# HKUST-Aerial-Robotics/MIND

Hardware: AMD Instinct MI355X
Metric: sim steps/sec (whole node) + scenario-tree nodes expanded/sec, AV2 demo scenes (higher is better)
Workload: dtype f32-class (bf16 hi+mid+lo split operands = 24 significand bits, six products, fp32 accumulate) pair kernel + ActorNet, f32 elsewhere in the predictor, f64 iLQR

## Files before the change

### mind_amd/csrc/actor_mfma_kernels.hip

```cpp
#include <hip/hip_runtime.h>
#include <stdint.h>

#define AM_T 1024
#ifdef MIND_ACTOR_TRACE
__device__ long long am_tr_[64];
__device__ int am_trn_;
#define AM_MARK() do { if (blockIdx.x == 0 && threadIdx.x == 0) { const long long n_ = clock64(); am_tr_[am_trn_ & 63] = n_; ++am_trn_; } } while (0)
#else
#define AM_MARK() do {} while (0)
#endif
#define AM_WAVES 16
#define AM_MAXT 2
#define AM_RSD(C) (3 * (C) / 2 + 4)
#define AM_BUF 2496
#define AM_XIN 0
#define AM_O0 1344
#define AM_FA (AM_O0 + 7 * AM_BUF)
#define AM_RED (AM_FA + 48 * AM_RSD(128))
#define AM_LDS_DWORDS (AM_RED + 64)

struct AmRes { const u32 *c1, *c2, *ds; const float *g1, *b1, *g2, *b2, *gd, *bd; };
struct AmLat { const u32 *w; const float *g, *b; };
struct AmW {
  AmRes res[9];
  AmLat lat[4];
};
typedef u32 u32x2 __attribute__((ext_vector_type(2)));

__device__ __forceinline__ float am_block_sum(float v, float *red, int flip) {
  v = wave_sum(v);
  float *r = red + (flip & 1) * 32;
  if ((threadIdx.x & 63) == 0) r[threadIdx.x >> 6] = v;
  __syncthreads();
  float s = 0.f;
#pragma unroll
  for (int w = 0; w < AM_WAVES; ++w) s += r[w];
  return s;
}

template <int NP>
__device__ __forceinline__ void am_store_split(u32 *rowp, int plane, const f32x4 &y) {
  u32x2 h, m, l;
  h[0] = pk_bf16(y[0], y[1]); h[1] = pk_bf16(y[2], y[3]);
  *(u32x2 *)rowp = h;
  if (NP == 1) return;
  const float r0 = y[0] - bf_lo_f32(h[0]), r1 = y[1] - bf_hi_f32(h[0]), r2 = y[2] - bf_lo_f32(h[1]), r3 = y[3] - bf_hi_f32(h[1]);
  m[0] = pk_bf16(r0, r1); m[1] = pk_bf16(r2, r3);
  *(u32x2 *)(rowp + plane) = m;
  l[0] = pk_bf16(r0 - bf_lo_f32(m[0]), r1 - bf_hi_f32(m[0])); l[1] = pk_bf16(r2 - bf_lo_f32(m[1]), r3 - bf_hi_f32(m[1]));
// ... 39 lines not shown
      const int row = t * STRIDE + dk - PAD;
      u32x4 bh = {0u, 0u, 0u, 0u}, bm = {0u, 0u, 0u, 0u}, bl = {0u, 0u, 0u, 0u};
      if (dk < KSZ && t < Tout && row >= 0 && row < Tin) {
        const u32 *bp = in + row * RSD + (ci >> 1);
        bh = *(const u32x4 *)bp;
        if (NP >= 3) bm = *(const u32x4 *)(bp + PLANE);
        if (NP == 6) bl = *(const u32x4 *)(bp + 2 * PLANE);
      }
      acc[i] = MFMA_BF(ah, bh, acc[i]);
      if (NP >= 3) {
        if (NP == 6) {
          corr = MFMA_BF(al, bh, corr);
          corr = MFMA_BF(ah, bl, corr);
          corr = MFMA_BF(am, bm, corr);
        }
        corr = MFMA_BF(am, bh, corr);
        corr = MFMA_BF(ah, bm, corr);
      }
    }
    if (NP >= 3) acc[i] += corr;
  }
}

template <int NP>
__device__ __forceinline__ void am_gn(f32x4 (&acc)[AM_MAXT], int Cout, int Tout, const float *__restrict__ g,
                                      const float *__restrict__ b, const u32 *resid, const float *up, bool relu, u32 *outs,
                                      float *outf, float *__restrict__ gout, float *red) {
  const int lane = threadIdx.x & 63, wave = threadIdx.x >> 6;
  const int r = lane & 15, q = lane >> 4;
  const int ntt = (Tout + 15) >> 4;
  const int tiles = (Cout >> 4) * ntt;
  const int RSD = AM_RSD(Cout), PLANE = Cout >> 1;
  f32x4 gg[AM_MAXT], bb[AM_MAXT];
  float s = 0.f;
#pragma unroll
  for (int i = 0; i < AM_MAXT; ++i) {
    const int ti = wave + AM_WAVES * i;
    if (ti >= tiles) continue;
    const int mt = ti / ntt, nt = ti - mt * ntt;
    gg[i] = *(const f32x4 *)(g + mt * 16 + q * 4);
    bb[i] = *(const f32x4 *)(b + mt * 16 + q * 4);
    if (nt * 16 + r < Tout) s += (acc[i][0] + acc[i][1]) + (acc[i][2] + acc[i][3]);
  }
  const float n = (float)(Cout * Tout);
  const float mean = am_block_sum(s, red, 0) / n;
  float v = 0.f;
// ... 56 lines not shown
  AM_MARK();
  const u32 *resid = in;
  if (DS) {
    am_conv<NP, LGCI, 1, STRIDE>(in, Tin, W.ds, Cout, Tout, acc);
    AM_MARK();
    am_gn<NP>(acc, Cout, Tout, W.gd, W.bd, nullptr, nullptr, false, t2, nullptr, nullptr, red);
    AM_MARK();
    resid = t2;
  }
  am_conv<NP, LGCO, 3, 1>(t1, Tout, W.c2, Cout, Tout, acc);
  AM_MARK();
  am_gn<NP>(acc, Cout, Tout, W.g2, W.b2, resid, nullptr, true, out, nullptr, nullptr, red);
  AM_MARK();
}

template <int NP, int LGC>
__device__ __forceinline__ void am_lateral(const u32 *src, int T, const AmLat &W, const float *up, float *dstf, u32 *dsts,
                                           float *red) {
  f32x4 acc[AM_MAXT];
  am_conv<NP, LGC, 3, 1>(src, T, W.w, 128, T, acc);
  AM_MARK();
  am_gn<NP>(acc, 128, T, W.g, W.b, nullptr, up, false, dsts, dstf, nullptr, red);
  AM_MARK();
}

template <int NP>
__global__ __launch_bounds__(AM_T) void k_actor_mfma(const float *__restrict__ actors , int n_actors,
                                                     float *__restrict__ out , AmW W) {
  extern __shared__ __attribute__((aligned(16))) u32 smu[];
  u32 *xin = smu + AM_XIN;
  u32 *o0 = smu + AM_O0, *o1 = o0 + AM_BUF, *o2 = o1 + AM_BUF, *o3 = o2 + AM_BUF;
  u32 *ta = o3 + AM_BUF, *tb = ta + AM_BUF, *tc = tb + AM_BUF;
  u32 *fa = smu + AM_FA;
  float *red = (float *)(smu + AM_RED);
  const int tid = threadIdx.x;
  const int a = blockIdx.x;
  if (a >= n_actors) return;
  if (tid < 48 * 8) {
    const int t = tid >> 3, c = (tid & 7) * 2;
    const float v0 = c < 14 ? actors[((size_t)a * 14 + c) * 48 + t] : 0.f;
    const float v1 = c + 1 < 14 ? actors[((size_t)a * 14 + c + 1) * 48 + t] : 0.f;
    u32 *p = xin + t * AM_RSD(16) + (c >> 1);
    const u32 h = pk_bf16(v0, v1);
    const float r0 = v0 - bf_lo_f32(h), r1 = v1 - bf_hi_f32(h);
    const u32 m = pk_bf16(r0, r1);
    p[0] = h; p[8] = m; p[16] = pk_bf16(r0 - bf_lo_f32(m), r1 - bf_hi_f32(m));
  }
  __syncthreads();
#ifdef MIND_ACTOR_TRACE
  if (blockIdx.x == 0 && tid == 0) am_trn_ = 0;
#endif
  AM_MARK();
  am_res<NP, 4, 5, 1, true>(xin, 48, W.res[0], ta, tb, tc, red);
  am_res<NP, 5, 5, 1, false>(ta, 48, W.res[1], o0, tb, tc, red);
  am_res<NP, 5, 6, 2, true>(o0, 48, W.res[2], ta, tb, tc, red);
  am_res<NP, 6, 6, 1, false>(ta, 24, W.res[3], o1, tb, tc, red);
  am_res<NP, 6, 7, 2, true>(o1, 24, W.res[4], ta, tb, tc, red);
  am_res<NP, 7, 7, 1, false>(ta, 12, W.res[5], o2, tb, tc, red);
  am_res<NP, 7, 8, 2, true>(o2, 12, W.res[6], ta, tb, tc, red);
  am_res<NP, 8, 8, 1, false>(ta, 6, W.res[7], o3, tb, tc, red);
  am_lateral<NP, 8>(o3, 6, W.lat[3], nullptr, (float *)ta, nullptr, red);
  am_lateral<NP, 7>(o2, 12, W.lat[2], (const float *)ta, (float *)tb, nullptr, red);
  am_lateral<NP, 6>(o1, 24, W.lat[1], (const float *)tb, (float *)o2, nullptr, red);
  am_lateral<NP, 5>(o0, 48, W.lat[0], (const float *)o2, nullptr, fa, red);
  {
    const AmRes &R = W.res[8];
    f32x4 acc[AM_MAXT];
    am_conv<NP, 7, 3, 1>(fa, 48, R.c1, 128, 48, acc);
    AM_MARK();
    am_gn<NP>(acc, 128, 48, R.g1, R.b1, nullptr, nullptr, true, o0, nullptr, nullptr, red);
    AM_MARK();
    am_conv<NP, 7, 3, 1>(o0, 48, R.c2, 128, 48, acc);
    AM_MARK();
    am_gn<NP>(acc, 128, 48, R.g2, R.b2, fa, nullptr, true, nullptr, nullptr, out + (size_t)a * 128, red);
    AM_MARK();
  }
#ifdef MIND_ACTOR_TRACE
  if (blockIdx.x == 0 && tid == 0) {
    printf("[k_actor_mfma<%d>] cycles conv/gn per stage:", NP);
    for (int q = 1; q < am_trn_ && q < 64; ++q) printf(" %lld", am_tr_[q] - am_tr_[q - 1]);
    printf("\n");
  }
#endif
}
extern "C" size_t mind_actor_mfma_lds_bytes() { return (size_t)AM_LDS_DWORDS * sizeof(u32); }
```

### mind_amd/csrc/mind_hip.hip

```cpp
#include <hip/hip_runtime.h>

#include <cmath>
#include <cstdarg>
#include <cstdio>
#include <cstdlib>
#include <algorithm>
#include <cstring>
#include <map>
#include <string>
#include <thread>
#include <atomic>
#include <functional>
#include <vector>

#include "../../include/mind_hip.h"
#include "encdec_kernels.hip"
#include "fusion_kernels.hip"
#include "pair_bf16_kernels.hip"
#include "pair_tile_kernels.hip"
#include "pair_tile6_kernels.hip"
#include "token_mfma_kernels.hip"
#include "actor_mfma_kernels.hip"
#include "actor_lw_kernels.hip"
#include "token_lw_kernels.hip"
// ... 239 lines not shown
  (void)hipFuncSetAttribute((const void *)k_pair_t6<1>, hipFuncAttributeMaxDynamicSharedMemorySize, (int)mind_pair_bf_lds_bytes());
  if (const char *te = getenv("MIND_PAIR_TILE")) c->pt.pair_tile = !(te[0] == '0');
  if (const char *xe = getenv("MIND_XCD_ORDER")) c->pt.xcd_order = !(xe[0] == '0');

  if (const char *pe = getenv("MIND_PAIR_PREC")) {
    const std::string v = pe;
    if (v == "f32" || v == "0") c->pair_prec = 0;
    else if (v == "bf16x3" || v == "1") c->pair_prec = 1;
    else if (v == "bf16" || v == "2") c->pair_prec = 2;
    else if (v == "bf16x6" || v == "3") c->pair_prec = 3;
  }
  (void)hipFuncSetAttribute((const void *)k_actor_net, hipFuncAttributeMaxDynamicSharedMemorySize, (int)mind_actor_lds_bytes());
  (void)hipFuncSetAttribute((const void *)k_actor_mfma<3>, hipFuncAttributeMaxDynamicSharedMemorySize, (int)mind_actor_mfma_lds_bytes());
  (void)hipFuncSetAttribute((const void *)k_actor_mfma<6>, hipFuncAttributeMaxDynamicSharedMemorySize, (int)mind_actor_mfma_lds_bytes());
  (void)hipFuncSetAttribute((const void *)k_dec_actor_mfma<1>, hipFuncAttributeMaxDynamicSharedMemorySize, (int)mind_dec_actor_mfma_lds_bytes());
  (void)hipFuncSetAttribute((const void *)k_dec_actor_mfma<3>, hipFuncAttributeMaxDynamicSharedMemorySize, (int)mind_dec_actor_mfma_lds_bytes());
  (void)hipFuncSetAttribute((const void *)k_dec_actor_mfma<6>, hipFuncAttributeMaxDynamicSharedMemorySize, (int)mind_dec_actor_mfma_lds_bytes());
  if (const char *se = getenv("MIND_ACTOR_SPLIT")) c->pt.actor_np = atoi(se) == 3 ? 3 : 6;
  (void)hipFuncSetAttribute((const void *)k_actor_mfma<1>, hipFuncAttributeMaxDynamicSharedMemorySize, (int)mind_actor_mfma_lds_bytes());
  if (const char *me = getenv("MIND_ENC_MFMA")) c->pt.enc_mfma = !(me[0] == '0');
  if (const char *me = getenv("MIND_ACTOR_F32")) c->pt.actor_f32 = !(me[0] == '0');
  if (const char *me = getenv("MIND_ACTOR_F32_MIN")) c->pt.actor_f32_min = atoi(me);
  if (const char *me = getenv("MIND_ACTOR_LW_MIN")) c->pt.actor_lw_min = atoi(me);
  lw_set_attributes();
  (void)hipFuncSetAttribute((const void *)k_actor_f32<1>, hipFuncAttributeMaxDynamicSharedMemorySize, (int)mind_actor_f32_lds_bytes(1));
  (void)hipFuncSetAttribute((const void *)k_actor_f32<2>, hipFuncAttributeMaxDynamicSharedMemorySize, (int)mind_actor_f32_lds_bytes(2));
  if (const char *de = getenv("MIND_DEC_MFMA_MIN")) c->pt.dec_mfma_min = atoi(de);
  if (const char *oe = getenv("MIND_DEC_OVERLAP")) c->pt.dec_overlap = !(oe[0] == '0');
  (void)hipFuncSetAttribute((const void *)k_ilqr<true, 0>, hipFuncAttributeMaxDynamicSharedMemorySize, (int)il_lds_bytes(0));
  (void)hipFuncSetAttribute((const void *)k_ilqr<false, 1>, hipFuncAttributeMaxDynamicSharedMemorySize, (int)il_lds_bytes(0));
  (void)hipFuncSetAttribute((const void *)k_ilqr<false, 0>, hipFuncAttributeMaxDynamicSharedMemorySize, (int)il_lds_bytes(0));
  (void)hipFuncSetAttribute((const void *)k_ilqr<false, 2>, hipFuncAttributeMaxDynamicSharedMemorySize, (int)il_lds_bytes(0));
  if (const char *te = getenv("MIND_TOK_MFMA")) c->pt.tok_mfma = !(te[0] == '0');
  if (const char *te = getenv("MIND_TOK_SMALL_MAX")) c->pt.tok_small_max = atoi(te);
  if (const char *te = getenv("MIND_TOK_MERGE")) c->pt.tok_merge = !(te[0] == '0');
  if (const char *te = getenv("MIND_DEC_MW")) c->pt.dec_mw = !(te[0] == '0');
  if (const char *te = getenv("MIND_DEC_CLS_SIDE")) c->pt.dec_cls_side = !(te[0] == '0');
  if (const char *te = getenv("MIND_TOK_BF_MIN_N")) c->pt.tok_bf_min_n = atoi(te);
  if (const char *te = getenv("MIND_TOK_LW_MIN_N")) c->pt.tok_lw_min_n = atoi(te);
  if (const char *te = getenv("MIND_TOK_LW_MIN")) c->pt.tok_lw_min = atoi(te);
  if (const char *te = getenv("MIND_TGT_SIDE")) c->pt.tgt_side = !(te[0] == '0');
  if (const char *te = getenv("MIND_PL_TAB_SIDE")) c->pl_tab_side = !(te[0] == '0');
  (void)hipFuncSetAttribute((const void *)k_token_mfma<0>, hipFuncAttributeMaxDynamicSharedMemorySize, (int)mind_token_mfma_lds_bytes());
  (void)hipFuncSetAttribute((const void *)k_token_mfma<1>, hipFuncAttributeMaxDynamicSharedMemorySize, (int)mind_token_mfma_lds_bytes());
  if (const char *ce = getenv("MIND_PLAN_CHUNK_MB")) { const long v = atol(ce); if (v > 0) c->plan_chunk_mb = v; }
  if (const char *we = getenv("MIND_TAB_SMALL")) c->tab_small = atoi(we) != 0;
// ... 470 lines not shown
  WeightBlob &B = c->blob;
  B.host.clear();
  B.off.clear();
  auto lin_ln = [&](const std::string &key, const std::string &p, int idx, int n_out, int n_in) {
    B.add(key + ".W", transpose(sd.get(p + "." + std::to_string(idx) + ".weight", (int64_t)n_out * n_in), n_out, n_in));
    B.add(key + ".b", vec(sd.get(p + "." + std::to_string(idx) + ".bias", n_out), n_out));
    B.add(key + ".g", vec(sd.get(p + "." + std::to_string(idx + 1) + ".weight", n_out), n_out));
    B.add(key + ".be", vec(sd.get(p + "." + std::to_string(idx + 1) + ".bias", n_out), n_out));
  };
  lin_ln("lane.proj", "lane_net.proj", 0, 128, 16);
  for (int b = 0; b < 2; ++b) {
    std::string p = "lane_net.aggre" + std::to_string(b + 1), k = "lane.a" + std::to_string(b);
    lin_ln(k + ".f10", p + ".fc1", 0, 128, 128);
    lin_ln(k + ".f13", p + ".fc1", 3, 128, 128);
    lin_ln(k + ".f20", p + ".fc2", 0, 128, 256);
    lin_ln(k + ".f23", p + ".fc2", 3, 128, 128);
    B.add(k + ".ng", vec(sd.get(p + ".norm.weight", 128), 128));
    B.add(k + ".nb", vec(sd.get(p + ".norm.bias", 128), 128));
  }
  {
    const int chans[4] = {32, 64, 128, 256};
    int n_in = 14;
    int ri = 0;
    auto res = [&](const std::string &p, int ci, int co, bool ds) {
      std::string k = "act.r" + std::to_string(ri++);
      B.add(k + ".c1", conv_t(sd.get(p + ".conv1.weight", (int64_t)co * ci * 3), co, ci, 3));
      B.add(k + ".c2", conv_t(sd.get(p + ".conv2.weight", (int64_t)co * co * 3), co, co, 3));
      B.add(k + ".c1B", pack_conv_frag(sd.get(p + ".conv1.weight", (int64_t)co * ci * 3), co, ci, 3));
      B.add(k + ".c2B", pack_conv_frag(sd.get(p + ".conv2.weight", (int64_t)co * co * 3), co, co, 3));
      B.add(k + ".c1F", pack_conv_f32(sd.get(p + ".conv1.weight", (int64_t)co * ci * 3), co, ci, 3));
      B.add(k + ".c2F", pack_conv_f32(sd.get(p + ".conv2.weight", (int64_t)co * co * 3), co, co, 3));
      B.add(k + ".g1", vec(sd.get(p + ".bn1.weight", co), co));
      B.add(k + ".b1", vec(sd.get(p + ".bn1.bias", co), co));
      B.add(k + ".g2", vec(sd.get(p + ".bn2.weight", co), co));
      B.add(k + ".b2", vec(sd.get(p + ".bn2.bias", co), co));
      if (ds) {
        B.add(k + ".ds", conv_t(sd.get(p + ".downsample.0.weight", (int64_t)co * ci), co, ci, 1));
        B.add(k + ".dsB", pack_conv_frag(sd.get(p + ".downsample.0.weight", (int64_t)co * ci), co, ci, 1));
        B.add(k + ".dsF", pack_conv_f32(sd.get(p + ".downsample.0.weight", (int64_t)co * ci), co, ci, 1));
        B.add(k + ".gd", vec(sd.get(p + ".downsample.1.weight", co), co));
        B.add(k + ".bd", vec(sd.get(p + ".downsample.1.bias", co), co));
      }
    };
    for (int g = 0; g < 4; ++g) {
      res("actor_net.groups." + std::to_string(g) + ".0", n_in, chans[g], true);
      res("actor_net.groups." + std::to_string(g) + ".1", chans[g], chans[g], false);
      n_in = chans[g];
    }
    res("actor_net.output", 128, 128, false);
    for (int g = 0; g < 4; ++g) {
      std::string p = "actor_net.lateral." + std::to_string(g), k = "act.lat" + std::to_string(g);
      B.add(k + ".W", conv_t(sd.get(p + ".conv.weight", (int64_t)128 * chans[g] * 3), 128, chans[g], 3));
      B.add(k + ".WB", pack_conv_frag(sd.get(p + ".conv.weight", (int64_t)128 * chans[g] * 3), 128, chans[g], 3));
      B.add(k + ".WF", pack_conv_f32(sd.get(p + ".conv.weight", (int64_t)128 * chans[g] * 3), 128, chans[g], 3));
      B.add(k + ".g", vec(sd.get(p + ".norm.weight", 128), 128));
      B.add(k + ".b", vec(sd.get(p + ".norm.bias", 128), 128));
    }
  }
  lin_ln("fus.pa", "fusion_net.proj_actor", 0, 128, 128);
  lin_ln("fus.pl", "fusion_net.proj_lane", 0, 128, 128);
  B.add("fus.pa.WM", pack_afrag(sd.get("fusion_net.proj_actor.0.weight", 128 * 128), 128));
  B.add("fus.pl.WM", pack_afrag(sd.get("fusion_net.proj_lane.0.weight", 128 * 128), 128));
  B.add("fus.pa.WB", pack_tok_bfrag(sd.get("fusion_net.proj_actor.0.weight", 128 * 128), 128));
  B.add("fus.pl.WB", pack_tok_bfrag(sd.get("fusion_net.proj_lane.0.weight", 128 * 128), 128));
  {
    const float *W = sd.get("fusion_net.proj_rpe_scene.0.weight", 128 * 5);
    const float *b = sd.get("fusion_net.proj_rpe_scene.0.bias", 128);
    const float *g = sd.get("fusion_net.proj_rpe_scene.1.weight", 128);
    const float *be = sd.get("fusion_net.proj_rpe_scene.1.bias", 128);
    std::vector<float> t(1024, 0.f);
    if (W && b && g && be)
      for (int ch = 0; ch < 32; ++ch)
        for (int w = 0; w < 4; ++w) {
          const int f = 4 * ch + w;
          for (int k = 0; k < 5; ++k) t[ch * 32 + k * 4 + w] = W[f * 5 + k];
          t[ch * 32 + 20 + w] = b[f];
          t[ch * 32 + 24 + w] = g[f];
          t[ch * 32 + 28 + w] = be[f];
        }
    B.add("fus.rtab", t);
// ... 146 lines not shown
  ActorW &aw = c->actorW;
  for (int r = 0; r < 9; ++r) {
    std::string k = "act.r" + std::to_string(r);
    aw.res[r].c1 = P(k + ".c1"); aw.res[r].g1 = P(k + ".g1"); aw.res[r].b1 = P(k + ".b1");
    aw.res[r].c2 = P(k + ".c2"); aw.res[r].g2 = P(k + ".g2"); aw.res[r].b2 = P(k + ".b2");
    aw.res[r].ds = P(k + ".ds"); aw.res[r].gd = P(k + ".gd"); aw.res[r].bd = P(k + ".bd");
  }
  for (int g = 0; g < 4; ++g) {
    std::string k = "act.lat" + std::to_string(g);
    aw.latW[g] = P(k + ".W"); aw.latG[g] = P(k + ".g"); aw.latB[g] = P(k + ".b");
  }
  AmW &bw = c->actorBW;
  for (int r = 0; r < 9; ++r) {
    std::string k = "act.r" + std::to_string(r);
    AmRes &R = bw.res[r];
    R.c1 = (const u32 *)P(k + ".c1B"); R.c2 = (const u32 *)P(k + ".c2B"); R.ds = (const u32 *)P(k + ".dsB");
    R.g1 = aw.res[r].g1; R.b1 = aw.res[r].b1; R.g2 = aw.res[r].g2; R.b2 = aw.res[r].b2;
    R.gd = aw.res[r].gd; R.bd = aw.res[r].bd;
  }
  for (int g = 0; g < 4; ++g) {
    bw.lat[g].w = (const u32 *)P("act.lat" + std::to_string(g) + ".WB");
    bw.lat[g].g = aw.latG[g]; bw.lat[g].b = aw.latB[g];
  }
  AfW &fw = c->actorFW;
  for (int r = 0; r < 9; ++r) {
    std::string k = "act.r" + std::to_string(r);
    AfRes &R = fw.res[r];
    R.c1 = P(k + ".c1F"); R.c2 = P(k + ".c2F"); R.ds = P(k + ".dsF");
    R.g1 = aw.res[r].g1; R.b1 = aw.res[r].b1; R.g2 = aw.res[r].g2; R.b2 = aw.res[r].b2;
    R.gd = aw.res[r].gd; R.bd = aw.res[r].bd;
  }
  for (int g = 0; g < 4; ++g) {
    fw.lat[g].w = P("act.lat" + std::to_string(g) + ".WF");
    fw.lat[g].g = aw.latG[g]; fw.lat[g].b = aw.latB[g];
  }
  c->rtab = P("fus.rtab");
  for (int L = 0; L < 6; ++L) {
    std::string k = "fus.L" + std::to_string(L);
    c->WAe[L] = P(k + ".WAe");
    c->WAp[L] = P(k + ".WAp");
    c->WBe[L] = (const u32 *)P(k + ".WBe");
    c->WBp[L] = (const u32 *)P(k + ".WBp");
    c->WLe[L] = (const u32 *)P(k + ".WLe");
    c->WLp[L] = (const u32 *)P(k + ".WLp");
    c->vtab[L] = P(k + ".vtab");
  }
// ... 447 lines not shown
```

### mind_amd/csrc/pred_choice.h

```cpp
#pragma once
#include <cstring>
#include <vector>

struct PredTuning {
  bool pair_tile = true;
  bool xcd_order = true;
  bool enc_mfma = true;
  int actor_np = 6;
  bool actor_f32 = true;
  int actor_f32_min = 1 << 30, actor_f32_pair_min = 1 << 30;
  int actor_lw_min = 1 << 30, actor_lw_chunk = 0;
  bool tok_mfma = false;
  int tok_bf_min_n = 0;
  int tok_lw_min_n = 1 << 30, tok_lw_min = 1 << 30, tok_lw_chunk = 0;
  bool tok_merge = true;
  int tok_small_max = 2048;
  int dec_mfma_min = 1 << 30;
  bool dec_overlap = true;
  bool dec_mw = false;
  bool dec_cls_side = false;
  bool tgt_side = true;
};

static bool pred_tuning_set(PredTuning &t, const char *name, int value) {
  const auto is = [name](const char *k) { return strcmp(name, k) == 0; };
  if (is("dec_mfma_min")) t.dec_mfma_min = value;
  else if (is("enc_mfma")) t.enc_mfma = value != 0;
  else if (is("actor_f32")) t.actor_f32 = value != 0;
  else if (is("actor_f32_min")) t.actor_f32_min = value;
  else if (is("actor_f32_pair_min")) t.actor_f32_pair_min = value;
  else if (is("actor_lw_min")) t.actor_lw_min = value;
  else if (is("actor_lw_chunk")) t.actor_lw_chunk = value < 0 ? 0 : value;
  else if (is("actor_split")) t.actor_np = value == 3 ? 3 : 6;
  else if (is("xcd_order")) t.xcd_order = value != 0;
  else if (is("pair_tile")) t.pair_tile = value != 0;
  else if (is("dec_overlap")) t.dec_overlap = value != 0;
  else if (is("tok_mfma")) t.tok_mfma = value != 0;
  else if (is("tok_small_max")) t.tok_small_max = value;
  else if (is("tok_merge")) t.tok_merge = value != 0;
  else if (is("dec_mw")) t.dec_mw = value != 0;
  else if (is("dec_cls_side")) t.dec_cls_side = value != 0;
  else if (is("tok_bf_min_n")) t.tok_bf_min_n = value;
  else if (is("tok_lw_min_n")) t.tok_lw_min_n = value;
  else if (is("tok_lw_min")) t.tok_lw_min = value;
  else if (is("tok_lw_chunk")) t.tok_lw_chunk = value < 0 ? 0 : value;
  else if (is("tgt_side")) t.tgt_side = value != 0;
  else return false;
  return true;
}

static inline int pred_mfma_parts(const PredTuning &t, int pair_prec) {
  return (pair_prec == 3 || (pair_prec == 1 && t.actor_np == 6)) ? 6 : (pair_prec == 1 ? 3 : 1);
}

static inline bool pred_edge_tiled(const PredTuning &t, int pair_prec) { return pair_prec == 3 || (pair_prec != 0 && t.pair_tile); }

static inline int pred_edge_pair_bytes(const PredTuning &t, int pair_prec) { return pred_edge_tiled(t, pair_prec) && pair_prec == 2 ? 256 : 512; }

enum PredActorForm { PRED_ACTOR_VALU = 0, PRED_ACTOR_F32 = 1, PRED_ACTOR_MFMA = 2, PRED_ACTOR_LW = 3 };
enum PredPairFamily { PRED_PAIR_F32 = 0, PRED_PAIR_BF = 1, PRED_PAIR_T = 2, PRED_PAIR_T6 = 3 };
enum PredDecActor { PRED_DEC_ONE = 0, PRED_DEC_SPLIT = 1, PRED_DEC_MFMA = 2 };

struct PredTokRun {
  int t0, n, kind;
  bool layerwise;
  bool small, merged;
};

struct PredChoice {
  int np = 1;
  int actor_form = PRED_ACTOR_VALU, actor_arg = 0, actor_grid = 0, actor_chunk = 0, actor_chunks = 1, actor_launches = 1;
  int qsplit = 0, qk_stride = 1024;
  bool tiled = false, edge_bf16 = false;
  std::vector<PredTokRun> tok_runs;
  int tok_chunk = 0;
  bool tok_lw = false;
  int last_tok_chunks = 0;
  int pair_family = PRED_PAIR_F32, pair_np = 0;
  bool l5_jobs5 = false;
  int xcd_lanes = 1, xcd_lanes5 = 1;
  int dec_actor = PRED_DEC_ONE;
  bool fp32_dec = true, split_dec = false, want_mw = false, cls_side = false;
  int mw_blocks = 0;
  bool tgt_wait_first = false;
};

static PredChoice pred_choose(const PredTuning &t, int pair_prec, int n_cu, bool have_side, int n_scenes, const int *scene_actors, const int *scene_lanes) {
  PredChoice ch;
  int A = 0;
  for (int b = 0; b < n_scenes; ++b) A += scene_actors[b];
  ch.np = pred_mfma_parts(t, pair_prec);

  ch.actor_grid = A;
  if (t.actor_f32 && A >= (pair_prec == 0 ? t.actor_f32_pair_min : t.actor_f32_min)) {
    ch.actor_form = PRED_ACTOR_F32; ch.actor_arg = 2; ch.actor_grid = (A + 1) / 2;
  } else if (pair_prec == 0 && t.actor_f32 && t.enc_mfma) {
    ch.actor_form = PRED_ACTOR_F32; ch.actor_arg = 1;
  } else if (pair_prec == 0 || !t.enc_mfma) {
    ch.actor_form = PRED_ACTOR_VALU;
  } else if (A >= t.actor_lw_min) {
    ch.actor_form = PRED_ACTOR_LW; ch.actor_arg = ch.np;
    ch.actor_chunk = t.actor_lw_chunk > 0 ? t.actor_lw_chunk : LW_CHUNK;
    ch.actor_chunks = (A + ch.actor_chunk - 1) / ch.actor_chunk;
    ch.actor_grid = ch.actor_chunks;
    ch.actor_launches = ch.actor_chunks * (1 + 2 * LW_NSTAGE);
  } else {
    ch.actor_form = PRED_ACTOR_MFMA; ch.actor_arg = ch.np;
  }

  ch.qsplit = pair_prec == 3 ? 48 : pair_prec != 0 ? 16 : 0;
  ch.qk_stride = pair_prec == 3 ? P6_QK_STRIDE : 1024;
  ch.tiled = pred_edge_tiled(t, pair_prec);
  ch.edge_bf16 = pred_edge_pair_bytes(t, pair_prec) == 256;

  ch.tok_chunk = t.tok_lw_chunk > 0 ? t.tok_lw_chunk : TL_CHUNK;
  long long njobs = 0, njobs5 = 0;
  int t0 = 0;
  for (int b = 0; b < n_scenes; ++b) {
    const int N = scene_actors[b] + scene_lanes[b] + 1;
    const int kind = t.tok_mfma ? 1 : (pair_prec != 0 && pair_prec != 3 && t.tok_bf_min_n > 0 && N >= t.tok_bf_min_n) ? 2 : N >= t.tok_lw_min_n ? 1 : 0;
    if (!ch.tok_runs.empty() && ch.tok_runs.back().kind == kind) ch.tok_runs.back().n += N;
    else ch.tok_runs.push_back({t0, N, kind, false, false, false});
    t0 += N;
    njobs += (long long)N * pair_column_splits(N);
    njobs5 += (long long)(scene_actors[b] + 1) * pair_column_splits(N);
  }
  for (PredTokRun &r : ch.tok_runs) {
    r.layerwise = r.kind == 1 && r.n >= t.tok_lw_min;
    r.small = r.kind == 0 && r.n <= t.tok_small_max;
    r.merged = r.small && t.tok_merge;
// ... 22 lines not shown
```

### mind_amd/csrc/predict.hip

```cpp
__global__ void k_tokpos(const TokMeta *__restrict__ meta, int n_tok, const float *__restrict__ actr,
                         const float *__restrict__ avec, const float *__restrict__ lctr,
                         const float *__restrict__ lvec, float *__restrict__ tokpos) {
  const int t = blockIdx.x * blockDim.x + threadIdx.x;
  if (t >= n_tok) return;
  const TokMeta m = meta[t];
  float4 o = make_float4(0.f, 0.f, 0.f, 0.f);
  if (m.type == 0 && actr) o = make_float4(actr[m.src * 2], actr[m.src * 2 + 1], avec[m.src * 2], avec[m.src * 2 + 1]);
  if (m.type == 1 && lctr) o = make_float4(lctr[m.src * 2], lctr[m.src * 2 + 1], lvec[m.src * 2], lvec[m.src * 2 + 1]);
  ((float4 *)tokpos)[t] = o;
}

struct PairTables {
  std::vector<TokMeta> meta;
  std::vector<PairJob> jobs, jobs5;
  std::vector<int> actor_row, actor_scene, cls_row, scene_n;
  long long edge_pairs = 0, edge_pairs_t = 0;
  int ntok = 0, slot = 0;
  double pairs_full = 0, pairs_l5 = 0;
};

static void pair_tables_build(int Bn, const int *scene_actors, const int *scene_lanes, bool xcd_order, int n_cu, PairTables &T) {
  int A = 0;
  for (int b = 0; b < Bn; ++b) A += scene_actors[b];
  T.actor_row.assign(A, 0); T.actor_scene.assign(A, 0); T.cls_row.assign(Bn, 0); T.scene_n.assign(Bn, 0);
// ... 197 lines not shown
  const int A = p.A;
  const dim3 grid(ch.actor_grid);
  switch (ch.actor_form) {
  case PRED_ACTOR_F32:
    if (ch.actor_arg == 2) hipLaunchKernelGGL(k_actor_f32<2>, grid, dim3(AF_T), mind_actor_f32_lds_bytes(2), p.st, actors, A, actor_feat, c->actorFW);
    else hipLaunchKernelGGL(k_actor_f32<1>, grid, dim3(AF_T), mind_actor_f32_lds_bytes(1), p.st, actors, A, actor_feat, c->actorFW);
    break;
  case PRED_ACTOR_VALU:
    hipLaunchKernelGGL(k_actor_net, grid, dim3(AT), mind_actor_lds_bytes(), p.st, actors, A, actor_feat, c->actorW);
    break;
  case PRED_ACTOR_LW: {
    int rc;
    if ((rc = ensure_exact(c, c->actor_lw_arena, lw_arena_bytes(ch.actor_chunk), "the layer-wise ActorNet's arena"))) return rc;
    lw_build_plan(A, ch.actor_chunk, c->actor_lw_plan);
    u32 *arena = (u32 *)c->actor_lw_arena.p;
    const int nl = ch.np == 6 ? lw_run<6>(c->actor_lw_plan, p.st, arena, actors, actor_feat, c->actorBW)
                 : ch.np == 3 ? lw_run<3>(c->actor_lw_plan, p.st, arena, actors, actor_feat, c->actorBW)
                              : lw_run<1>(c->actor_lw_plan, p.st, arena, actors, actor_feat, c->actorBW);
    if (nl < 0) return fail(c, MIND_ESTATE, "layer-wise ActorNet: a stage has no kernel");
    c->last_actor_lw = 1; c->last_actor_launches = nl; c->last_actor_chunks = ch.actor_chunks;
    break;
  }
  default:
    if (ch.np == 6) hipLaunchKernelGGL(k_actor_mfma<6>, grid, dim3(AM_T), mind_actor_mfma_lds_bytes(), p.st, actors, A, actor_feat, c->actorBW);
    else if (ch.np == 3) hipLaunchKernelGGL(k_actor_mfma<3>, grid, dim3(AM_T), mind_actor_mfma_lds_bytes(), p.st, actors, A, actor_feat, c->actorBW);
    else hipLaunchKernelGGL(k_actor_mfma<1>, grid, dim3(AM_T), mind_actor_mfma_lds_bytes(), p.st, actors, A, actor_feat, c->actorBW);
  }
  return MIND_OK;
}

static int pred_encoders(PredCall &p) {
  mind_ctx *c = p.c;
  const mind_scene_batch *in = p.in;
  hipStream_t st = p.st, ss = p.ss;
  const int Bn = p.Bn, Ltot = p.Ltot, ntok = p.ts->ntok;
  if (c->side) {
    HIPCHK(c, hipEventRecord(c->ev_main, st));
    HIPCHK(c, hipStreamWaitEvent(c->side, c->ev_main, 0));
  }
  const bool act_timed = c->profiling && !c->ev_defer;
  if (act_timed && !c->ev_act0) {
    HIPCHK(c, hipEventCreate(&c->ev_act0));
    HIPCHK(c, hipEventCreate(&c->ev_act1));
  }
  c->last_actor_lw = 0; c->last_actor_launches = 1; c->last_actor_chunks = 1; c->actor_ms = 0.f;
  if (act_timed) HIPCHK(c, hipEventRecord(c->ev_act0, st));
  int rc;
// ... 285 lines not shown
```

Baseline: 1791.

## Prefetch ActorNet weight fragments ahead across conv stages and stage norm affines in LDS

```diff
diff --git a/mind_amd/csrc/actor_mfma_kernels.hip b/mind_amd/csrc/actor_mfma_kernels.hip
--- a/mind_amd/csrc/actor_mfma_kernels.hip
+++ b/mind_amd/csrc/actor_mfma_kernels.hip
@@ -24,7 +24,19 @@
 struct AmW {
   AmRes res[9];
   AmLat lat[4];
+  const float *aff;
 };
+__host__ __device__ constexpr int am_res_ch(int r) { return r == 8 ? 128 : 32 << (r >> 1); }
+__host__ __device__ constexpr bool am_res_ds(int r) { return r < 8 && !(r & 1); }
+__host__ __device__ constexpr int am_aff_res(int r) {
+  int o = 0;
+  for (int i = 0; i < r; ++i) o += am_res_ch(i) * (am_res_ds(i) ? 6 : 4);
+  return o;
+}
+__host__ __device__ constexpr int am_aff_lat(int g) { return am_aff_res(9) + 256 * g; }
+#define AM_AFF AM_LDS_DWORDS
+#define AM_AFF_FLOATS (am_aff_lat(4))
+#define AM_AH_LDS_DWORDS (AM_AFF + AM_AFF_FLOATS)
 typedef u32 u32x2 __attribute__((ext_vector_type(2)));
 
 __device__ __forceinline__ float am_block_sum(float v, float *red, int flip) {
@@ -110,6 +122,94 @@
   }
 }
 
+#define AM_AHD 3
+template <int NP> struct AmFr { u32x4 h, m, l; };
+template <int NP>
+__device__ __forceinline__ void am_fr_load(AmFr<NP> &f, const u32 *__restrict__ p) {
+  f.h = *(const u32x4 *)p;
+  if (NP >= 3) f.m = *(const u32x4 *)(p + 256);
+  if (NP == 6) f.l = *(const u32x4 *)(p + 512);
+}
+template <int NP, int KS>
+__device__ __forceinline__ void am_fr_req(AmFr<NP> &f, const u32 *__restrict__ Wf, int tiles, int ntt, int s) {
+  const int i = s / KS, ks = s - i * KS;
+  const int ti = (threadIdx.x >> 6) + AM_WAVES * i;
+  if (i < AM_MAXT && ti < tiles) am_fr_load<NP>(f, Wf + ((size_t)(ti / ntt) * KS + ks) * 768 + (threadIdx.x & 63) * 4);
+}
+template <int NP, int LGC, int KSZ>
+__device__ __forceinline__ void am_conv_pre(const u32 *__restrict__ Wf, int Cout, int Tout, AmFr<NP> (&fr)[AM_AHD]) {
+  constexpr int KS = (KSZ * (1 << LGC) + 31) / 32;
+  const int ntt = (Tout + 15) >> 4;
+#pragma unroll
+  for (int d = 0; d < AM_AHD; ++d) am_fr_req<NP, KS>(fr[d], Wf, (Cout >> 4) * ntt, ntt, d);
+}
+template <int NP, int LGC, int KSZ, int STRIDE>
+__device__ __forceinline__ void am_kstep(const AmFr<NP> &a, const u32 *in, int Tin, int Tout, int t, int q, int ks, f32x4 &acc,
+                                         f32x4 &corr) {
+  constexpr int CP = 1 << LGC, RSD = AM_RSD(CP), PLANE = CP / 2, PAD = (KSZ - 1) / 2;
+  const int k0 = ks * 32 + q * 8;
+  const int dk = k0 >> LGC, ci = k0 & (CP - 1);
+  const int row = t * STRIDE + dk - PAD;
+  u32x4 bh = {0u, 0u, 0u, 0u}, bm = {0u, 0u, 0u, 0u}, bl = {0u, 0u, 0u, 0u};
+  if (dk < KSZ && t < Tout && row >= 0 && row < Tin) {
+    const u32 *bp = in + row * RSD + (ci >> 1);
+    bh = *(const u32x4 *)bp;
+    if (NP >= 3) bm = *(const u32x4 *)(bp + PLANE);
+    if (NP == 6) bl = *(const u32x4 *)(bp + 2 * PLANE);
+  }
+  acc = MFMA_BF(a.h, bh, acc);
+  if (NP >= 3) {
+    if (NP == 6) {
+      corr = MFMA_BF(a.l, bh, corr);
+      corr = MFMA_BF(a.h, bl, corr);
+      corr = MFMA_BF(a.m, bm, corr);
+    }
+    corr = MFMA_BF(a.m, bh, corr);
+    corr = MFMA_BF(a.h, bm, corr);
+  }
+}
+template <int NP, int LGC, int KSZ, int STRIDE>
+__device__ __forceinline__ void am_conv_ah(const u32 *in, int Tin, const u32 *__restrict__ Wf, int Cout, int Tout,
+                                           f32x4 (&acc)[AM_MAXT], AmFr<NP> (&fr)[AM_AHD]) {
+  constexpr int KS = (KSZ * (1 << LGC) + 31) / 32;
+  constexpr int ROLL = KS > 6 ? KS - 6 : 0;
+  static_assert((KS <= 6 || KS % 6 == 0) && 6 % AM_AHD == 0, "a rolled k-loop takes six k-steps per trip");
+  const int lane = threadIdx.x & 63, wave = threadIdx.x >> 6;
+  const int r = lane & 15, q = lane >> 4;
+  const int ntt = (Tout + 15) >> 4;
+  const int tiles = (Cout >> 4) * ntt;
+#pragma unroll
+  for (int i = 0; i < AM_MAXT; ++i) {
+    acc[i] = (f32x4){0.f, 0.f, 0.f, 0.f};
+    const int ti = wave + AM_WAVES * i;
+    if (ti >= tiles) continue;
+    const int mt = ti / ntt, nt = ti - mt * ntt;
+    const int t = nt * 16 + r;
+    const u32 *wp = Wf + (size_t)mt * KS * 768 + lane * 4;
+    f32x4 corr = {0.f, 0.f, 0.f, 0.f};
+    for (int k6 = 0; k6 < ROLL; k6 += 6) {
+#pragma unroll
+      for (int u = 0; u < 6; ++u) {
+        am_kstep<NP, LGC, KSZ, STRIDE>(fr[u % AM_AHD], in, Tin, Tout, t, q, k6 + u, acc[i], corr);
+        am_fr_load<NP>(fr[u % AM_AHD], wp + (size_t)(k6 + u + AM_AHD) * 768);
+      }
+    }
+#pragma unroll
+    for (int ks = ROLL; ks < KS; ++ks) {
+      const int s = i * KS + ks;
+      am_kstep<NP, LGC, KSZ, STRIDE>(fr[s % AM_AHD], in, Tin, Tout, t, q, ks, acc[i], corr);
+      am_fr_req<NP, KS>(fr[s % AM_AHD], Wf, tiles, ntt, s + AM_AHD);
+    }
+    if (NP >= 3) acc[i] += corr;
+  }
+#pragma unroll
+  for (int d = 0; d < AM_AHD; ++d) {
+    asm volatile("" ::"v"(fr[d].h));
+    if (NP >= 3) asm volatile("" ::"v"(fr[d].m));
+    if (NP == 6) asm volatile("" ::"v"(fr[d].l));
+  }
+}
+
 template <int NP>
 __device__ __forceinline__ void am_gn(f32x4 (&acc)[AM_MAXT], int Cout, int Tout, const float *__restrict__ g,
                                       const float *__restrict__ b, const u32 *resid, const float *up, bool relu, u32 *outs,
@@ -212,6 +312,21 @@
   AM_MARK();
   am_gn<NP>(acc, 128, T, W.g, W.b, nullptr, up, false, dsts, dstf, nullptr, red);
   AM_MARK();
+}
+
+__device__ __forceinline__ void am_input(const float *__restrict__ actors, int a, u32 *xin) {
+  const int tid = threadIdx.x;
+  if (tid < 48 * 8) {
+    const int t = tid >> 3, c = (tid & 7) * 2;
+    const float v0 = c < 14 ? actors[((size_t)a * 14 + c) * 48 + t] : 0.f;
+    const float v1 = c + 1 < 14 ? actors[((size_t)a * 14 + c + 1) * 48 + t] : 0.f;
+    u32 *p = xin + t * AM_RSD(16) + (c >> 1);
+    const u32 h = pk_bf16(v0, v1);
+    const float r0 = v0 - bf_lo_f32(h), r1 = v1 - bf_hi_f32(h);
+    const u32 m = pk_bf16(r0, r1);
+    p[0] = h; p[8] = m; p[16] = pk_bf16(r0 - bf_lo_f32(m), r1 - bf_hi_f32(m));
+  }
+  __syncthreads();
 }
 
 template <int NP>
@@ -226,17 +341,7 @@
   const int tid = threadIdx.x;
   const int a = blockIdx.x;
   if (a >= n_actors) return;
-  if (tid < 48 * 8) {
-    const int t = tid >> 3, c = (tid & 7) * 2;
-    const float v0 = c < 14 ? actors[((size_t)a * 14 + c) * 48 + t] : 0.f;
-    const float v1 = c + 1 < 14 ? actors[((size_t)a * 14 + c + 1) * 48 + t] : 0.f;
-    u32 *p = xin + t * AM_RSD(16) + (c >> 1);
-    const u32 h = pk_bf16(v0, v1);
-    const float r0 = v0 - bf_lo_f32(h), r1 = v1 - bf_hi_f32(h);
-    const u32 m = pk_bf16(r0, r1);
-    p[0] = h; p[8] = m; p[16] = pk_bf16(r0 - bf_lo_f32(m), r1 - bf_hi_f32(m));
-  }
-  __syncthreads();
+  am_input(actors, a, xin);
 #ifdef MIND_ACTOR_TRACE
   if (blockIdx.x == 0 && tid == 0) am_trn_ = 0;
 #endif
@@ -273,4 +378,107 @@
   }
 #endif
 }
-extern "C" size_t mind_actor_mfma_lds_bytes() { return (size_t)AM_LDS_DWORDS * sizeof(u32); }
+
+template <int NP, int LGCI, int LGCO, int STRIDE, bool DS, class Next>
+__device__ __forceinline__ void am_res_ah(const u32 *in, int Tin, const AmRes &W, const float *aff ,
+                                          u32 *out, u32 *t1, u32 *t2, float *red, AmFr<NP> (&fr)[AM_AHD], Next next) {
+  constexpr int Cout = 1 << LGCO;
+  const int Tout = Tin / STRIDE;
+  f32x4 acc[AM_MAXT];
+  am_conv_ah<NP, LGCI, 3, STRIDE>(in, Tin, W.c1, Cout, Tout, acc, fr);
+  AM_MARK();
+  if (DS) am_conv_pre<NP, LGCI, 1>(W.ds, Cout, Tout, fr);
+  else am_conv_pre<NP, LGCO, 3>(W.c2, Cout, Tout, fr);
+  am_gn<NP>(acc, Cout, Tout, aff, aff + Cout, nullptr, nullptr, true, t1, nullptr, nullptr, red);
+  AM_MARK();
+  const u32 *resid = in;
+  if constexpr (DS) {
+    am_conv_ah<NP, LGCI, 1, STRIDE>(in, Tin, W.ds, Cout, Tout, acc, fr);
+    AM_MARK();
+    am_conv_pre<NP, LGCO, 3>(W.c2, Cout, Tout, fr);
+    am_gn<NP>(acc, Cout, Tout, aff + 4 * Cout, aff + 5 * Cout, nullptr, nullptr, false, t2, nullptr, nullptr, red);
+    AM_MARK();
+    resid = t2;
+  }
+  am_conv_ah<NP, LGCO, 3, 1>(t1, Tout, W.c2, Cout, Tout, acc, fr);
+  AM_MARK();
+  next(fr);
+  am_gn<NP>(acc, Cout, Tout, aff + 2 * Cout, aff + 3 * Cout, resid, nullptr, true, out, nullptr, nullptr, red);
+  AM_MARK();
+}
+
+template <int NP, int LGC, class Next>
+__device__ __forceinline__ void am_lateral_ah(const u32 *src, int T, const AmLat &W, const float *aff, const float *up, float *dstf,
+                                              u32 *dsts, float *red, AmFr<NP> (&fr)[AM_AHD], Next next) {
+  f32x4 acc[AM_MAXT];
+  am_conv_ah<NP, LGC, 3, 1>(src, T, W.w, 128, T, acc, fr);
+  AM_MARK();
+  next(fr);
+  am_gn<NP>(acc, 128, T, aff, aff + 128, nullptr, up, false, dsts, dstf, nullptr, red);
+  AM_MARK();
+}
+
+#define AM_NEXT(LGC, WF, CO, TO) [&](AmFr<NP> (&f)[AM_AHD]) { am_conv_pre<NP, LGC, 3>(WF, CO, TO, f); }
+
+template <int NP>
+__global__ __launch_bounds__(AM_T) void k_actor_mfma_ah(const float *__restrict__ actors , int n_actors,
+                                                        float *__restrict__ out , AmW W) {
+  extern __shared__ __attribute__((aligned(16))) u32 smu[];
+  u32 *xin = smu + AM_XIN;
+  u32 *o0 = smu + AM_O0, *o1 = o0 + AM_BUF, *o2 = o1 + AM_BUF, *o3 = o2 + AM_BUF;
+  u32 *ta = o3 + AM_BUF, *tb = ta + AM_BUF, *tc = tb + AM_BUF;
+  u32 *fa = smu + AM_FA;
+  float *red = (float *)(smu + AM_RED);
+  const int tid = threadIdx.x;
+  const int a = blockIdx.x;
+  if (a >= n_actors) return;
+  const float *aff = (const float *)(smu + AM_AFF);
+  constexpr int NA4 = AM_AFF_FLOATS / 4;
+  static_assert(NA4 > AM_T && NA4 <= 2 * AM_T, "two float4 of the affine table per thread");
+  const f32x4 af0 = ((const f32x4 *)W.aff)[tid];
+  f32x4 af1 = {0.f, 0.f, 0.f, 0.f};
+  if (tid + AM_T < NA4) af1 = ((const f32x4 *)W.aff)[tid + AM_T];
+  AmFr<NP> fr[AM_AHD];
+  am_conv_pre<NP, 4, 3>(W.res[0].c1, 32, 48, fr);
+  am_input(actors, a, xin);
+  ((f32x4 *)(smu + AM_AFF))[tid] = af0;
+  if (tid + AM_T < NA4) ((f32x4 *)(smu + AM_AFF))[tid + AM_T] = af1;
+#ifdef MIND_ACTOR_TRACE
+  if (blockIdx.x == 0 && tid == 0) am_trn_ = 0;
+#endif
+  AM_MARK();
+  am_res_ah<NP, 4, 5, 1, true>(xin, 48, W.res[0], aff + am_aff_res(0), ta, tb, tc, red, fr, AM_NEXT(5, W.res[1].c1, 32, 48));
+  am_res_ah<NP, 5, 5, 1, false>(ta, 48, W.res[1], aff + am_aff_res(1), o0, tb, tc, red, fr, AM_NEXT(5, W.res[2].c1, 64, 24));
+  am_res_ah<NP, 5, 6, 2, true>(o0, 48, W.res[2], aff + am_aff_res(2), ta, tb, tc, red, fr, AM_NEXT(6, W.res[3].c1, 64, 24));
+  am_res_ah<NP, 6, 6, 1, false>(ta, 24, W.res[3], aff + am_aff_res(3), o1, tb, tc, red, fr, AM_NEXT(6, W.res[4].c1, 128, 12));
+  am_res_ah<NP, 6, 7, 2, true>(o1, 24, W.res[4], aff + am_aff_res(4), ta, tb, tc, red, fr, AM_NEXT(7, W.res[5].c1, 128, 12));
+  am_res_ah<NP, 7, 7, 1, false>(ta, 12, W.res[5], aff + am_aff_res(5), o2, tb, tc, red, fr, AM_NEXT(7, W.res[6].c1, 256, 6));
+  am_res_ah<NP, 7, 8, 2, true>(o2, 12, W.res[6], aff + am_aff_res(6), ta, tb, tc, red, fr, AM_NEXT(8, W.res[7].c1, 256, 6));
+  am_res_ah<NP, 8, 8, 1, false>(ta, 6, W.res[7], aff + am_aff_res(7), o3, tb, tc, red, fr, AM_NEXT(8, W.lat[3].w, 128, 6));
+  am_lateral_ah<NP, 8>(o3, 6, W.lat[3], aff + am_aff_lat(3), nullptr, (float *)ta, nullptr, red, fr, AM_NEXT(7, W.lat[2].w, 128, 12));
+  am_lateral_ah<NP, 7>(o2, 12, W.lat[2], aff + am_aff_lat(2), (const float *)ta, (float *)tb, nullptr, red, fr, AM_NEXT(6, W.lat[1].w, 128, 24));
+  am_lateral_ah<NP, 6>(o1, 24, W.lat[1], aff + am_aff_lat(1), (const float *)tb, (float *)o2, nullptr, red, fr, AM_NEXT(5, W.lat[0].w, 128, 48));
+  am_lateral_ah<NP, 5>(o0, 48, W.lat[0], aff + am_aff_lat(0), (const float *)o2, nullptr, fa, red, fr, AM_NEXT(7, W.res[8].c1, 128, 48));
+  {
+    const AmRes &R = W.res[8];
+    f32x4 acc[AM_MAXT];
+    am_conv_ah<NP, 7, 3, 1>(fa, 48, R.c1, 128, 48, acc, fr);
+    AM_MARK();
+    am_conv_pre<NP, 7, 3>(R.c2, 128, 48, fr);
+    am_gn<NP>(acc, 128, 48, aff + am_aff_res(8), aff + am_aff_res(8) + 128, nullptr, nullptr, true, o0, nullptr, nullptr, red);
+    AM_MARK();
+    am_conv_ah<NP, 7, 3, 1>(o0, 48, R.c2, 128, 48, acc, fr);
+    AM_MARK();
+    am_gn<NP>(acc, 128, 48, aff + am_aff_res(8) + 256, aff + am_aff_res(8) + 384, fa, nullptr, true, nullptr, nullptr, out + (size_t)a * 128, red);
+    AM_MARK();
+  }
+#ifdef MIND_ACTOR_TRACE
+  if (blockIdx.x == 0 && tid == 0) {
+    printf("[k_actor_mfma_ah<%d>] cycles conv/gn per stage:", NP);
+    for (int q = 1; q < am_trn_ && q < 64; ++q) printf(" %lld", am_tr_[q] - am_tr_[q - 1]);
+    printf("\n");
+  }
+#endif
+}
+#undef AM_NEXT
+extern "C" size_t mind_actor_mfma_lds_bytes() { return (size_t)AM_AH_LDS_DWORDS * sizeof(u32); }
diff --git a/mind_amd/csrc/mind_hip.hip b/mind_amd/csrc/mind_hip.hip
--- a/mind_amd/csrc/mind_hip.hip
+++ b/mind_amd/csrc/mind_hip.hip
@@ -285,6 +285,10 @@
   if (const char *me = getenv("MIND_ACTOR_F32")) c->pt.actor_f32 = !(me[0] == '0');
   if (const char *me = getenv("MIND_ACTOR_F32_MIN")) c->pt.actor_f32_min = atoi(me);
   if (const char *me = getenv("MIND_ACTOR_LW_MIN")) c->pt.actor_lw_min = atoi(me);
+  (void)hipFuncSetAttribute((const void *)k_actor_mfma_ah<6>, hipFuncAttributeMaxDynamicSharedMemorySize, (int)mind_actor_mfma_lds_bytes());
+  (void)hipFuncSetAttribute((const void *)k_actor_mfma_ah<3>, hipFuncAttributeMaxDynamicSharedMemorySize, (int)mind_actor_mfma_lds_bytes());
+  (void)hipFuncSetAttribute((const void *)k_actor_mfma_ah<1>, hipFuncAttributeMaxDynamicSharedMemorySize, (int)mind_actor_mfma_lds_bytes());
+  if (const char *me = getenv("MIND_ACTOR_AHEAD")) c->pt.actor_ahead = !(me[0] == '0');
   lw_set_attributes();
   (void)hipFuncSetAttribute((const void *)k_actor_f32<1>, hipFuncAttributeMaxDynamicSharedMemorySize, (int)mind_actor_f32_lds_bytes(1));
   (void)hipFuncSetAttribute((const void *)k_actor_f32<2>, hipFuncAttributeMaxDynamicSharedMemorySize, (int)mind_actor_f32_lds_bytes(2));
@@ -801,7 +805,13 @@
     const int chans[4] = {32, 64, 128, 256};
     int n_in = 14;
     int ri = 0;
+    std::vector<float> aff(AM_AFF_FLOATS, 0.f);
+    auto put = [&](int o, const float *v, int n) { if (v) std::copy(v, v + n, aff.begin() + o); };
     auto res = [&](const std::string &p, int ci, int co, bool ds) {
+      const int ao = am_aff_res(ri);
+      put(ao, sd.get(p + ".bn1.weight", co), co); put(ao + co, sd.get(p + ".bn1.bias", co), co);
+      put(ao + 2 * co, sd.get(p + ".bn2.weight", co), co); put(ao + 3 * co, sd.get(p + ".bn2.bias", co), co);
+      if (ds) { put(ao + 4 * co, sd.get(p + ".downsample.1.weight", co), co); put(ao + 5 * co, sd.get(p + ".downsample.1.bias", co), co); }
       std::string k = "act.r" + std::to_string(ri++);
       B.add(k + ".c1", conv_t(sd.get(p + ".conv1.weight", (int64_t)co * ci * 3), co, ci, 3));
       B.add(k + ".c2", conv_t(sd.get(p + ".conv2.weight", (int64_t)co * co * 3), co, co, 3));
@@ -834,7 +844,9 @@
       B.add(k + ".WF", pack_conv_f32(sd.get(p + ".conv.weight", (int64_t)128 * chans[g] * 3), 128, chans[g], 3));
       B.add(k + ".g", vec(sd.get(p + ".norm.weight", 128), 128));
       B.add(k + ".b", vec(sd.get(p + ".norm.bias", 128), 128));
-    }
+      put(am_aff_lat(g), sd.get(p + ".norm.weight", 128), 128); put(am_aff_lat(g) + 128, sd.get(p + ".norm.bias", 128), 128);
+    }
+    B.add("act.aff", aff);
   }
   lin_ln("fus.pa", "fusion_net.proj_actor", 0, 128, 128);
   lin_ln("fus.pl", "fusion_net.proj_lane", 0, 128, 128);
@@ -1027,6 +1039,7 @@
     bw.lat[g].w = (const u32 *)P("act.lat" + std::to_string(g) + ".WB");
     bw.lat[g].g = aw.latG[g]; bw.lat[g].b = aw.latB[g];
   }
+  bw.aff = P("act.aff");
   AfW &fw = c->actorFW;
   for (int r = 0; r < 9; ++r) {
     std::string k = "act.r" + std::to_string(r);
diff --git a/mind_amd/csrc/pred_choice.h b/mind_amd/csrc/pred_choice.h
--- a/mind_amd/csrc/pred_choice.h
+++ b/mind_amd/csrc/pred_choice.h
@@ -10,6 +10,7 @@
   bool actor_f32 = true;
   int actor_f32_min = 1 << 30, actor_f32_pair_min = 1 << 30;
   int actor_lw_min = 1 << 30, actor_lw_chunk = 0;
+  bool actor_ahead = true;
   bool tok_mfma = false;
   int tok_bf_min_n = 0;
   int tok_lw_min_n = 1 << 30, tok_lw_min = 1 << 30, tok_lw_chunk = 0;
@@ -30,6 +31,7 @@
   else if (is("actor_f32_min")) t.actor_f32_min = value;
   else if (is("actor_f32_pair_min")) t.actor_f32_pair_min = value;
   else if (is("actor_lw_min")) t.actor_lw_min = value;
+  else if (is("actor_ahead")) t.actor_ahead = value != 0;
   else if (is("actor_lw_chunk")) t.actor_lw_chunk = value < 0 ? 0 : value;
   else if (is("actor_split")) t.actor_np = value == 3 ? 3 : 6;
   else if (is("xcd_order")) t.xcd_order = value != 0;
@@ -70,6 +72,7 @@
 struct PredChoice {
   int np = 1;
   int actor_form = PRED_ACTOR_VALU, actor_arg = 0, actor_grid = 0, actor_chunk = 0, actor_chunks = 1, actor_launches = 1;
+  bool actor_ahead = false;
   int qsplit = 0, qk_stride = 1024;
   bool tiled = false, edge_bf16 = false;
   std::vector<PredTokRun> tok_runs;
@@ -105,7 +108,7 @@
     ch.actor_grid = ch.actor_chunks;
     ch.actor_launches = ch.actor_chunks * (1 + 2 * LW_NSTAGE);
   } else {
-    ch.actor_form = PRED_ACTOR_MFMA; ch.actor_arg = ch.np;
+    ch.actor_form = PRED_ACTOR_MFMA; ch.actor_arg = ch.np; ch.actor_ahead = t.actor_ahead;
   }
 
   ch.qsplit = pair_prec == 3 ? 48 : pair_prec != 0 ? 16 : 0;
diff --git a/mind_amd/csrc/predict.hip b/mind_amd/csrc/predict.hip
--- a/mind_amd/csrc/predict.hip
+++ b/mind_amd/csrc/predict.hip
@@ -243,7 +243,11 @@
     break;
   }
   default:
-    if (ch.np == 6) hipLaunchKernelGGL(k_actor_mfma<6>, grid, dim3(AM_T), mind_actor_mfma_lds_bytes(), p.st, actors, A, actor_feat, c->actorBW);
+    if (ch.actor_ahead) {
+      if (ch.np == 6) hipLaunchKernelGGL(k_actor_mfma_ah<6>, grid, dim3(AM_T), mind_actor_mfma_lds_bytes(), p.st, actors, A, actor_feat, c->actorBW);
+      else if (ch.np == 3) hipLaunchKernelGGL(k_actor_mfma_ah<3>, grid, dim3(AM_T), mind_actor_mfma_lds_bytes(), p.st, actors, A, actor_feat, c->actorBW);
+      else hipLaunchKernelGGL(k_actor_mfma_ah<1>, grid, dim3(AM_T), mind_actor_mfma_lds_bytes(), p.st, actors, A, actor_feat, c->actorBW);
+    } else if (ch.np == 6) hipLaunchKernelGGL(k_actor_mfma<6>, grid, dim3(AM_T), mind_actor_mfma_lds_bytes(), p.st, actors, A, actor_feat, c->actorBW);
     else if (ch.np == 3) hipLaunchKernelGGL(k_actor_mfma<3>, grid, dim3(AM_T), mind_actor_mfma_lds_bytes(), p.st, actors, A, actor_feat, c->actorBW);
     else hipLaunchKernelGGL(k_actor_mfma<1>, grid, dim3(AM_T), mind_actor_mfma_lds_bytes(), p.st, actors, A, actor_feat, c->actorBW);
   }
```

After: 1810 (median of 2 runs). About the same (+1.1%).
